# tonyzyl/ladcast

Hardware: AMD Instinct MI355X
Metric: ensemble-member-steps/sec (higher is better)
Workload: dtype f32

## Files before the change

include/ladcast_hip.h:

```cpp
#ifndef LADCAST_HIP_H
#define LADCAST_HIP_H

#ifdef __cplusplus
extern "C" {
#endif

#define LDC_ABI_VERSION 5

#define LDC_OK 0
#define LDC_ERR_ARG (-1)
#define LDC_ERR_ALIGN (-2)
#define LDC_ERR_UNSUPPORTED (-3)

enum ldc_act { LDC_ACT_NONE = 0, LDC_ACT_SILU = 1, LDC_ACT_GELU_TANH = 2, LDC_ACT_RELU = 3 };
#define LDC_ACT_IN_TIMESTEP_SINCOS 16

int ldc_abi_version(void);
const char* ldc_build_arch(void);

typedef struct ldc_gemm_desc {
  int M, N, K, batch;
  int lda, ldw, ldc, ldr;
  long long a_bs, c_bs, r_bs;
  int gate_bs;
// ... 100 lines not shown
int ldc_layernorm_mod(const float* x, float* y, int B, int rows, int D, int ldx, long long x_bs,
                      int ldy, long long y_bs, const float* scale, const float* shift, int mod_bs,
                      int mode, float eps, int out_split, void* stream);
int ldc_layernorm_mod2(const float* x, float* y, int B, int rows, int D, int ldx, long long x_bs,
                       int ldy, long long y_bs, const float* scale, const float* shift, int split_row,
                       const float* scale2, const float* shift2, int mod_bs, int mode, float eps,
                       int out_split, void* stream);

int ldc_mean_rows(const float* x, float* y, int B, int rows, int D, int ldx, long long x_bs, void* stream);
int ldc_mean_rows_split(const float* x, float* y, float* x_split, int B, int rows, int D, int ldx,
                        long long x_bs, int lds, long long s_bs, int fmt , void* stream);

int ldc_gate_residual(const float* resid, const float* y, const float* gate, float* out, int B,
                      int rows, int D, int ld_res, long long res_bs, int ld_y, long long y_bs,
                      int gate_bs, void* stream);
int ldc_gate_residual_layernorm(float* resid, const float* y, const float* gate, float* out, int B, int rows, int D, int ld_res,
                                long long res_bs, int ld_y, long long y_bs, int gate_bs, int ld_out, long long out_bs,
                                const float* weight, const float* bias, float eps, int out_split, void* stream);

int ldc_chan_to_token(const float* in, float* out, int B, int C, int N, int ldo, int fill_cols, void* stream);
int ldc_chan_to_token_split(const float* in, float* out, int B, int C, int N, int ldo, int fill_cols,
                            int out_split, void* stream);
int ldc_token_to_chan(const float* in, float* out, int B, int C, int N, int ldi, void* stream);

int ldc_timestep_embedding(const float* t, float* out, int n, void* stream);

int ldc_temb_modulate(float* temb, const float* te, int B, int D, int te_rows, void* stream);

int ldc_chan_affine(const float* x, float* y, const float* mean, const float* std_, float target_std,
                    long long outer, int C, long long inner, int inverse, void* stream);

int ldc_edm_scale_f64_to_f32(const double* x, double c_in, float* out, long long n, void* stream);
int ldc_edm_init_state(const float* noise, double sigma0, double* x, long long n, void* stream);
int ldc_edm_churn(const double* x_cur, const double* noise, double coef, double* x_hat, long long n, void* stream);
int ldc_edm_euler(const double* x_hat, const float* F, double c_skip, double c_out, double t_hat,
                  double dt, double* x_next, double* d_cur, long long n, void* stream);
int ldc_edm_heun(const double* x_hat, double* x_next, const float* F, const double* d_cur,
                 double c_skip, double c_out, double t_next, double dt, long long n, void* stream);
int ldc_f64_to_f32(const double* x, float* y, long long n, void* stream);
int ldc_dpm_step(const float* sample, const float* F, const float* m1, float* x0, float* prev,
                 float c_skip, float c_out, float a, float b, float inv_r0, int order, long long n,
                 void* stream);
int ldc_ddim_step(const float* sample, const float* F, const float* noise, float* x0, float* prev, float sqrt_alpha_t,
                  float sqrt_beta_t, float sqrt_alpha_prev, float dir_coef, float std_dev, float clip_range,
                  int prediction_type, int use_clipped_model_output, long long n, void* stream);
int ldc_ddpm_step(const float* sample, const float* F, const float* noise, float* x0, float* prev, float sqrt_alpha_t,
// ... 144 lines not shown
```

ladcast_amd/hip.py:

```python
from __future__ import annotations

import ctypes
import os
from ctypes import POINTER, Structure, c_char_p, c_double, c_float, c_int, c_longlong, c_void_p

import torch

_HERE = os.path.dirname(os.path.abspath(__file__))
LIB_PATH = os.environ.get("LDC_LIB_PATH") or os.path.join(_HERE, "libladcast_hip.so")

ACT_NONE, ACT_SILU, ACT_GELU_TANH, ACT_RELU = 0, 1, 2, 3
ACT_IN_TIMESTEP_SINCOS = 16
GEMM_A_SPLIT, GEMM_C_SPLIT, GEMM_BF16_1TERM = 1, 2, 4
GEMM_F32_REGSTAGE = 8
ATTN_OUT_SPLIT, ATTN_BF16_1TERM, ATTN_OUT_BF16 = 1, 2, 4
ABI_VERSION = 5
FMT_F32, FMT_SPLIT, FMT_BF16 = 0, 1, 2


class GemmDesc(Structure):
    _fields_ = [
        ("M", c_int), ("N", c_int), ("K", c_int), ("batch", c_int),
        ("lda", c_int), ("ldw", c_int), ("ldc", c_int), ("ldr", c_int),
        ("a_bs", c_longlong), ("c_bs", c_longlong), ("r_bs", c_longlong),
# ... 86 lines not shown
        "ldc_ensemble_scores_workspace_bytes": (L, [I, I, I]),
        "ldc_ensemble_scores": (I, [P, L, L, P, L, P, L, P, I, I, I, I, I, P, P, P, P, L, P]),
        "ldc_rollout_scores_workspace_bytes": (L, [I, I, I, I]),
        "ldc_rollout_scores": (I, [P, L, L, L, P, P, F, P, L, L, P, P, L, L, P, P, I, I, I, I, I, I, P, I, I, P, L, P]),
        "ldc_validation_scores_workspace_bytes": (L, [I, I, I, I]),
        "ldc_validation_scores": (I, [P, L, L, L, P, P, F, P, L, L, P, P, I, I, I, I, I, P, I, I, P, L, P]),
        "ldc_rollout_reliability_workspace_bytes": (L, [I, I, I, I, I]),
        "ldc_rollout_reliability": (I, [P, L, L, L, P, P, F, P, L, L, P, P, I, I, I, I, I, I, P, P, P, P, I, I, P, L, P]),
        "ldc_rollout_spectrum_workspace_bytes": (L, [I, I, I, I, I]),
        "ldc_rollout_spectrum": (I, [P, L, L, L, P, P, F, P, L, L, P, P, I, I, I, I, I, P, P, I, I, P, L, P]),
        "ldc_sizeof_products_desc": (I, []),
        "ldc_rollout_products": (I, [P, L, L, L, P, P, F, P, I, I, I, I, I, I, POINTER(ProductsDesc), P, P, P, P, I, I, P]),
        "ldc_sizeof_events_desc": (I, []),
        "ldc_rollout_events_workspace_bytes": (L, [I, I, I, I, I]),
        "ldc_rollout_events": (I, [P, L, L, L, P, P, F, P, L, L, P, P, L, L, P, P, I, I, I, I, I, POINTER(EventsDesc), P, P, P, I, I, P, L, P]),
        "ldc_layernorm_mod": (I, [P, P, I, I, I, I, L, I, L, P, P, I, I, F, I, P]),
        "ldc_layernorm_mod2": (I, [P, P, I, I, I, I, L, I, L, P, P, I, P, P, I, I, F, I, P]),
        "ldc_mean_rows": (I, [P, P, I, I, I, I, L, P]),
        "ldc_mean_rows_split": (I, [P, P, P, I, I, I, I, L, I, L, I, P]),
        "ldc_chan_to_token_split": (I, [P, P, I, I, I, I, I, I, P]),
        "ldc_gate_residual": (I, [P, P, P, P, I, I, I, I, L, I, L, I, P]),
        "ldc_chan_to_token": (I, [P, P, I, I, I, I, I, P]),
        "ldc_token_to_chan": (I, [P, P, I, I, I, I, P]),
        "ldc_timestep_embedding": (I, [P, P, I, P]),
        "ldc_temb_modulate": (I, [P, P, I, I, I, P]),
        "ldc_chan_affine": (I, [P, P, P, P, F, L, I, L, I, P]),
        "ldc_edm_scale_f64_to_f32": (I, [P, D, P, L, P]),
        "ldc_edm_init_state": (I, [P, D, P, L, P]),
        "ldc_edm_euler": (I, [P, P, D, D, D, D, P, P, L, P]),
        "ldc_edm_churn": (I, [P, P, c_double, P, L, P]),
        "ldc_edm_heun": (I, [P, P, P, P, D, D, D, D, L, P]),
        "ldc_f64_to_f32": (I, [P, P, L, P]),
        "ldc_dpm_step": (I, [P, P, P, P, P, F, F, F, F, F, I, L, P]),
        "ldc_ddim_step": (I, [P, P, P, P, P, F, F, F, F, F, F, I, I, L, P]),
        "ldc_ddpm_step": (I, [P, P, P, P, P, F, F, F, F, F, F, I, L, P]),
        "ldc_scale_f32": (I, [P, F, P, L, P]),
        "ldc_axpby_f32": (I, [P, F, P, F, P, L, P]),
        "ldc_edm_noise_inputs": (I, [P, P, P, P, P, P, I, L, P]),
        "ldc_edm_denoise": (I, [P, P, P, P, P, I, I, I, I, I, I, I, P]),
        "ldc_edm_denoise_loss": (I, [P, P, P, P, P, P, P, P, P, I, I, I, I, I, P]),
        "ldc_sphere_conv_nhwc": (I, [P, P, P, P, P, I, I, I, I, I, I, I, I, I, I, P]),
        "ldc_sphere_dwconv_nhwc": (I, [P, P, P, P, I, I, I, I, I, I, I, I, P]),
        "ldc_grouped_conv1x1_nhwc": (I, [P, P, P, L, I, I, I, P]),
        "ldc_relu_linear_attn_nhwc": (I, [P, P, I, I, I, I, I, F, P, L, P]),
        "ldc_relu_linear_attn_workspace_bytes": (L, [I, I, I]),
        "ldc_rmsnorm_rows": (I, [P, P, P, P, P, L, I, I, I, I, F, I, P]),
# ... 463 lines not shown
        _check(lib.ldc_mean_rows(_p(x), _p(y), B, rows, D, ldx, x_bs, _stream()), "ldc_mean_rows")
    else:
        _check(lib.ldc_mean_rows_split(_p(x), _p(y), _p(x_split), B, rows, D, ldx, x_bs, lds if lds is not None else ldx,
                                       s_bs if s_bs is not None else x_bs, int(fmt), _stream()), "ldc_mean_rows_split")


def gate_residual(resid, y, gate, out, *, B, rows, D, ld_res, res_bs, ld_y, y_bs, gate_bs):
    _dev(resid, y, gate, out)
    _check(lib.ldc_gate_residual(_p(resid), _p(y), _p(gate), _p(out), B, rows, D, ld_res, res_bs, ld_y, y_bs, gate_bs, _stream()),
           "ldc_gate_residual")


def chan_to_token(x, out, *, B, C, N, ldo, fill_cols=None, out_split=False):
    _dev(x, out)
    _check(lib.ldc_chan_to_token_split(_p(x), _p(out), B, C, N, ldo, ldo if fill_cols is None else fill_cols, int(out_split), _stream()),
           "ldc_chan_to_token")


def token_to_chan(x, out, *, B, C, N, ldi):
    _dev(x, out)
    _check(lib.ldc_token_to_chan(_p(x), _p(out), B, C, N, ldi, _stream()), "ldc_token_to_chan")


def timestep_embedding(t, out, n):
    _dev(t, out)
    _check(lib.ldc_timestep_embedding(_p(t), _p(out), n, _stream()), "ldc_timestep_embedding")


def temb_modulate(temb, te, *, B, D, te_rows):
    _dev(temb, te)
    _check(lib.ldc_temb_modulate(_p(temb), _p(te), B, D, te_rows, _stream()), "ldc_temb_modulate")


def chan_affine(x, y, mean, std, target_std, *, outer, C, inner, inverse):
    _dev(x, y, mean, std)
    _check(lib.ldc_chan_affine(_p(x), _p(y), _p(mean), _p(std), target_std, outer, C, inner, int(inverse), _stream()), "ldc_chan_affine")


TRACK_MAX_CHANNELS, TRACK_MAX_BOXES, TRACK_MAX_INNER, TRACK_MAX_GRID = 8, 8, 30, 1024


def _int_array(values):
    return (c_int * len(values))(*[int(v) for v in values])


def track_gather(x, out, channels, mean, std, *, sb, st, sc, B, T, HW, T_total, t_off, target_std=1.0):
# ... 239 lines not shown
```

ladcast_amd/models/LaDCast_3D_model.py:

```python
from __future__ import annotations

from types import SimpleNamespace
from typing import Optional, Tuple

import numpy as np
import torch
import torch.nn as nn

from .. import graphs, hip
from .embeddings import get_year_sincos_embedding, rope_tables_from_grid, rotary_1d
from .modeling_utils import ModelMixin


class _RMSNormP(nn.Module):
    def __init__(self, dim, eps):
        super().__init__()
        self.eps = eps
        self.weight = nn.Parameter(torch.ones(dim))

    def forward(self, x):
        var = x.to(torch.float32).pow(2).mean(-1, keepdim=True)
        return x * torch.rsqrt(var + self.eps) * self.weight


# ... 524 lines not shown
        C_out = cfg.out_channels or cfg.in_channels
        hidden_states = hidden_states.to(device=dev, dtype=torch.float32).contiguous()
        conditioning_tensors = conditioning_tensors.to(device=dev, dtype=torch.float32)
        if conditioning_tensors.shape[0] != B:
            conditioning_tensors = conditioning_tensors.expand(B, -1, -1, -1, -1)
        conditioning_tensors = conditioning_tensors.contiguous()
        timestep = timestep.to(device=dev, dtype=torch.float32).reshape(-1).contiguous()
        Bt = timestep.shape[0]
        if Bt not in (1, B):
            raise ValueError(f"timestep must have 1 or {B} entries, got {Bt}")
        te = None
        if time_elapsed is not None and self.time_elapsed_embed is not None:
            te = self._time_elapsed_embedding(time_elapsed, dev)
            if te.shape[0] not in (1, B):
                raise ValueError("time_elapsed must have 1 or batch entries")

        if conditioning is not None:
            pack, idx = conditioning
            if tuple(pack.shape) != (B,) + tuple(conditioning_tensors.shape[1:]) or not 0 <= idx < pack.levels:
                raise ValueError("`conditioning` was prepared for another batch / conditioning shape")
            out = self._main_device(hidden_states, pack, idx)
            return (out,) if not return_dict else SimpleNamespace(sample=out)
        if self.use_hip_graph:
            gkey = (B, Bt, C_in, R, T_in, Hh, Ww, None if te is None else (te.data_ptr(), te.shape[0]), bool(self.skip_unread_rows))
            inputs = [hidden_states, timestep, conditioning_tensors]
            ent = self._graphs.get(gkey)
            if ent is None:
                ent = self._graphs[gkey] = graphs.capture(lambda x, t, k: self._forward_device(x, t, k, te), inputs, dev, self.capture_stream())
            out = ent.replay(*inputs)
        else:
            out = self._forward_device(hidden_states, timestep, conditioning_tensors, te)
        if not return_dict:
            return (out,)
        return SimpleNamespace(sample=out)

    def time_elapsed_embedding(self, time_elapsed):
        if time_elapsed is None or self.time_elapsed_embed is None:
            return None
        if self._plan is None:
            self._build_plan()
        return self._time_elapsed_embedding(time_elapsed, self.device)

    def plan_identity(self):
        if self._plan is None:
            self._build_plan()
        return self._plan_gen

    def capture_stream(self):
        if self._capture_stream is None:
            self._capture_stream = torch.cuda.Stream(device=self.device)
        return self._capture_stream

    @torch.no_grad()
    def forward_launch_only(self, hidden_states, timestep, conditioning_tensors, te, conditioning=None):
        if self._plan is None:
            self._build_plan()
        if hidden_states.dtype != torch.float32 or not hidden_states.is_cuda or not hidden_states.is_contiguous():
            raise TypeError("forward_launch_only takes a contiguous fp32 device tensor (use forward() for anything else)")
        if conditioning is not None:
            return self._main_device(hidden_states, conditioning[0], conditioning[1])
        return self._forward_device(hidden_states, timestep.reshape(-1), conditioning_tensors, te)

    batch_conditioning = True
    skip_unread_rows = True
    COND_MAX_ROWS = 96

    @torch.no_grad()
    def prepare_conditioning(self, timesteps, conditioning_tensors, te=None):
        if self._plan is None:
            self._build_plan()
        dev = self.device
        timesteps = timesteps.to(device=dev, dtype=torch.float32).reshape(-1)
        conditioning_tensors = conditioning_tensors.to(device=dev, dtype=torch.float32)
        if conditioning_tensors.dim() != 5:
            raise ValueError("conditioning_tensors must be (B, C, T_in, h, w)")
        N, B = timesteps.shape[0], conditioning_tensors.shape[0]
        shape = tuple(conditioning_tensors.shape)
        per = max(1, self.COND_MAX_ROWS // B)
        if per >= N:
            pk = self._conditioning_device(timesteps.repeat_interleave(B).contiguous(),
                                           conditioning_tensors.unsqueeze(0).expand(N, *shape).reshape(N * B, *shape[1:]).contiguous(), te)
            return SimpleNamespace(ctx=pk.ctx, mods=pk.mods, shape=shape, levels=N)
        Nc, D, NM = shape[2] * shape[3] * shape[4] // self._patch_vol, self.inner_dim, self._plan.mod_w.shape[0]
        key = ("pack", N, B, Nc)
        if key not in self._ws:
            self._ws[key] = (torch.empty(N * B, Nc, D, device=dev, dtype=torch.float32), torch.empty(N * B, NM, device=dev, dtype=torch.float32))
        ctx, mods = self._ws[key]
# ... 126 lines not shown
        cfg = self.config
        D, H = self.inner_dim, cfg.num_attention_heads
        hidden_states = self._patches(hidden_states)
        B, C_in, R, Hh, Ww = hidden_states.shape
        T_in = pack.shape[2] // cfg.patch_size_t
        Nx, Nc = R * Hh * Ww, T_in * Hh * Ww
        S = Nx + Nc
        C_out = (cfg.out_channels or cfg.in_channels) * self._patch_vol
        kpad = max(plan.kx_pad, plan.kc_pad)
        key = (B, Nx, Nc, kpad)
        if key not in self._ws:
            self._ws[key] = _Workspace(dev, B, 1, Nx, Nc, D, kpad, C_out, 4)
        ws = self._ws[key]
        pc, ps, cc, cs, pk, ck, jk = self._rope_tables(R, T_in, Hh, Ww, dev)
        SD = S * D
        h_x, h_c = ws.h[:, :Nx], ws.h[:, Nx:]
        nh_x, nh_c = ws.nh[:, :Nx], ws.nh[:, Nx:]
        NM = plan.mod_w.shape[0]
        mods = pack.mods[idx * B : (idx + 1) * B]
        split = plan.split

        AS, CS, fmt, G, run, run1, run_qkv = self._launchers(plan)

        if split:
            KX = plan.kx_pad
            xtok = ws.xtok.view(-1)[: B * Nx * KX].view(B, Nx, KX)
            hip.chan_to_token(hidden_states, xtok, B=B, C=C_in, N=Nx, ldo=KX, fill_cols=KX, out_split=fmt)
            run1(xtok, plan.wx, h_x, M=Nx, N=D, K=KX, batch=B, a_bs=Nx * KX, c_bs=SD, bias=self.x_embedder.proj.bias, flags=AS)
        else:
            hip.chan_to_token(hidden_states, ws.xtok.view(-1)[: B * Nx * C_in].view(B, Nx, C_in), B=B, C=C_in, N=Nx, ldo=C_in)
            hip.gemm(ws.xtok, plan.wx, h_x, M=Nx, N=D, K=C_in, batch=B, a_bs=Nx * C_in, c_bs=SD, bias=self.x_embedder.proj.bias)
        h_c.copy_(pack.ctx[idx * B : (idx + 1) * B])

        kb_all = None
        if self.scale_attn_by_lat:
            if Hh * Ww != self.attn_lat_weights.numel():
                raise ValueError("scale_attn_by_lat is hard-wired to the 15 x 30 latent grid (models/LaDCast_3D_model.py:684-692)")
            kb_all = self._key_bias(R + T_in, dev)
        foreign = bool(self._foreign_processors())
        m_all = None
        if foreign:
            if split:
                raise NotImplementedError("a user-supplied attention processor runs on the fp32 path: call set_gemm_precision('fp32') "
                                          "(or change the attention arithmetic through the C ABI, include/ladcast_hip.h)")
            if torch.cuda.is_current_stream_capturing():
                raise NotImplementedError("a user-supplied attention processor cannot be captured into a hipGraph")
            if self.scale_attn_by_lat:
                w = self.attn_lat_weights.to(dev)
                m_all = w.repeat(1, 1, 1, T_in + R)


        def mod_of(linear, width):
            o = plan.mod_off[id(linear)]
            return mods[:, o : o + width]

        for blk in self.transformer_blocks:
            pa = plan.attn[id(blk.attn)]
            mx, mc = mod_of(blk.norm1.linear, 6 * D), mod_of(blk.norm1_context.linear, 6 * D)
            hip.layernorm_mod(ws.h, ws.nh, B=B, rows=S, D=D, ldx=D, x_bs=SD, ldy=D, y_bs=SD, scale=mx[:, D:], shift=mx, split_row=Nx, scale2=mc[:, D:], shift2=mc,
                              mod_bs=NM, mode=0, eps=1e-6, out_split=fmt)
            if blk.attn.foreign_processor is not None:
                a, ca = self._call_processor(blk.attn, nh_x, nh_c, m_all, (pc, ps), (cc, cs))
                a, ca = a.contiguous(), ca.contiguous()
                hip.gate_residual(h_x, a, mx[:, 2 * D :], h_x, B=B, rows=Nx, D=D, ld_res=D, res_bs=SD, ld_y=D, y_bs=Nx * D, gate_bs=NM)
                hip.gate_residual(h_c, ca, mc[:, 2 * D :], h_c, B=B, rows=Nc, D=D, ld_res=D, res_bs=SD, ld_y=D, y_bs=Nc * D, gate_bs=NM)
            else:
                nd = run_qkv([
                    G(nh_x, pa.wqkv, ws.qkv, M=Nx, N=3 * D, K=D, batch=B, a_bs=SD, c_bs=S * 3 * D, bias=pa.bqkv, flags=AS),
                    G(nh_c, pa.wqkv_c, ws.qkv[:, Nx:], M=Nc, N=3 * D, K=D, batch=B, a_bs=SD, c_bs=S * 3 * D, bias=pa.bqkv_c, flags=AS),
                ], [self._qkv_epi(blk.attn.norm_q, blk.attn.norm_k, pk), self._qkv_epi(blk.attn.norm_added_q, blk.attn.norm_added_k, None)])
                self._attention(ws, B, 0, Nx, Nc, ws.att, D, SD, (blk.attn.norm_q, blk.attn.norm_k, pc, ps),
                                (blk.attn.norm_added_q, blk.attn.norm_added_k, None, None), out_split=fmt, key_bias=kb_all, normed=nd)
                o, oc = blk.attn.to_out[0], blk.attn.to_add_out
                run([
                    G(ws.att, o.weight, h_x, M=Nx, N=D, K=D, batch=B, a_bs=SD, c_bs=SD, bias=o.bias, gate=mx[:, 2 * D :], gate_bs=NM, R=h_x, ldr=D, r_bs=SD, flags=AS),
                    G(ws.att[:, Nx:], oc.weight, h_c, M=Nc, N=D, K=D, batch=B, a_bs=SD, c_bs=SD, bias=oc.bias, gate=mc[:, 2 * D :], gate_bs=NM, R=h_c, ldr=D, r_bs=SD, flags=AS),
                ])
            hip.layernorm_mod(ws.h, ws.nh, B=B, rows=S, D=D, ldx=D, x_bs=SD, ldy=D, y_bs=SD, scale=mx[:, 4 * D :], shift=mx[:, 3 * D :], split_row=Nx,
                              scale2=mc[:, 4 * D :], shift2=mc[:, 3 * D :], mod_bs=NM, mode=0, eps=1e-7, out_split=fmt)
            up, down = [], []
            for (hs, nhs, rows, ff, mod, off) in ((h_x, nh_x, Nx, blk.ff, mx, 0), (h_c, nh_c, Nc, blk.ff_context, mc, Nx)):
                f0, f2 = ff.net[0].proj, ff.net[2]
                F = f0.weight.shape[0]
# ... 11 lines not shown
            mod = mod_of(blk.norm.linear, 3 * D)
            F = blk.proj_mlp.weight.shape[0]
            W5 = D + F
            cat_mlp = ws.cat.view(torch.bfloat16)[:, :, D:] if plan.one_term else ws.cat[:, :, D:]
            hip.layernorm_mod(ws.h, ws.nh, B=B, rows=S, D=D, ldx=D, x_bs=SD, ldy=D, y_bs=SD, scale=mod[:, D:], shift=mod, mod_bs=NM, mode=0, eps=1e-6, out_split=fmt)
            if blk.attn.foreign_processor is not None:
                run([G(ws.nh, blk.proj_mlp.weight, cat_mlp, M=S, N=F, K=D, batch=B, a_bs=SD, ldc=W5, c_bs=S * W5, bias=blk.proj_mlp.bias,
                       act=hip.ACT_GELU_TANH, flags=AS | CS)])
                a, ca = self._call_processor(blk.attn, ws.nh[:, :Nx], ws.nh[:, Nx:], m_all, (pc, ps), (cc, cs))
                ws.cat[:, :Nx, :D].copy_(a)
                ws.cat[:, Nx:, :D].copy_(ca)
            else:
                nd = run_qkv([
                    G(ws.nh, blk.proj_mlp.weight, cat_mlp, M=Mq, N=F, K=D, batch=B, a_bs=SD, ldc=W5, c_bs=S * W5, bias=blk.proj_mlp.bias, act=hip.ACT_GELU_TANH,
                      flags=AS | CS),
                    G(ws.nh, pa.wqkv, ws.qkv, M=S, N=3 * D, K=D, batch=B, a_bs=SD, c_bs=S * 3 * D, bias=pa.bqkv, flags=AS),
                ], [None, self._qkv_epi(blk.attn.norm_q, blk.attn.norm_k, jk)])
                self._attention(ws, B, 0, Nx, Nc, ws.cat, W5, S * W5, (blk.attn.norm_q, blk.attn.norm_k, pc, ps),
                                (blk.attn.norm_q, blk.attn.norm_k, cc, cs), out_split=fmt, key_bias=kb_all, normed=nd, Sq=None if Mq == S else Mq)
            run1(ws.cat, blk.proj_out.weight, ws.h, M=Mq, N=D, K=W5, batch=B, a_bs=S * W5, c_bs=SD, bias=blk.proj_out.bias,
                        gate=mod[:, 2 * D :], gate_bs=NM, R=ws.h, ldr=D, r_bs=SD, flags=AS)

        mo = mod_of(self.norm_out.linear, 2 * D)
        hip.layernorm_mod(h_x, nh_x, B=B, rows=Nx, D=D, ldx=D, x_bs=SD, ldy=D, y_bs=SD, scale=mo, shift=mo[:, D:], mod_bs=NM, mode=0, eps=1e-7, out_split=fmt)
        run1(nh_x, self.proj_out.weight, ws.otok, M=Nx, N=C_out, K=D, batch=B, a_bs=SD, c_bs=Nx * C_out, bias=self.proj_out.bias, flags=AS)
        out = torch.empty(B, C_out, R, Hh, Ww, device=dev, dtype=torch.float32)
        hip.token_to_chan(ws.otok, out, B=B, C=C_out, N=Nx, ldi=C_out)
        return self._unpatch(out, cfg.out_channels or cfg.in_channels)
```

ladcast_amd/pipelines/edm_sampler.py:

```python
from __future__ import annotations

from typing import List, Optional, Union

import numpy as np
import torch

from .. import graphs, hip
from .torch_utils import randn_tensor


@torch.no_grad()
def edm_AR_sampler(
    net,
    noise_scheduler,
    batch_size=1,
    return_seq_len=1,
    randn_like=torch.randn_like,
    num_inference_steps=18,
    S_churn=0,
    S_min=0,
    S_max=float("inf"),
    S_noise=0,
    deterministic=True,
    known_latents=None,
# ... 13 lines not shown
    shape = (batch_size, net.config.out_channels, return_seq_len, *known_latents.shape[-2:])
    latents = randn_tensor(shape, generator=generator, device=device, dtype=torch.float32).contiguous()
    noise_scheduler.set_timesteps(num_inference_steps, device=device)
    t_steps = noise_scheduler.sigmas
    c_noise_host = noise_scheduler.precondition_noise(t_steps[:-1])
    known = known_latents.to(device=device, dtype=torch.float32)
    if known.shape[0] != batch_size:
        known = known.expand(batch_size, *known.shape[1:])
    known = known.contiguous()

    chunk_graph = bool(getattr(net, "use_hip_graph", False)) and hasattr(net, "forward_launch_only") and hasattr(net, "_graphs")
    batched = bool(getattr(net, "batch_conditioning", False)) and hasattr(net, "prepare_conditioning")
    if not deterministic:
        out = torch.empty(shape, device=device, dtype=torch.float32)
        fwd = lambda x, t, k, te_: net(x, t, k, time_elapsed=timestamps).sample
        _heun_chunk_stochastic(fwd, noise_scheduler, t_steps, latents, known, out, shape, device, num_inference_steps, randn_like, S_churn, S_min,
                               S_max, S_noise)
        return out
    if chunk_graph:
        te = net.time_elapsed_embedding(timestamps)
        plan_id = net.plan_identity()
        key = (tuple(shape), tuple(known.shape), num_inference_steps, tuple(float(v) for v in t_steps.tolist()),
               None if te is None else (te.data_ptr(), tuple(te.shape)), str(device), plan_id, batched,
               bool(getattr(net, "skip_unread_rows", False)))
        prepare = net.prepare_conditioning if batched else None
        key = ("edm_chunk",) + key
        cache = net._graphs
        turn = cache.get(key + ("turn",), 0)
        cache[key + ("turn",)] = turn ^ 1

        def capture():
            st_out, cn = torch.empty(shape, device=device, dtype=torch.float32), c_noise_host.to(device)

            def chunk(lat, kn):
                _heun_chunk(net.forward_launch_only, noise_scheduler, t_steps, cn, lat, kn, te, st_out, shape, device, num_inference_steps, prepare)
                return st_out

            return graphs.capture(chunk, [latents, known], device, net.capture_stream(), keep=cn)

        for inst in (turn, turn ^ 1):
            if cache.get(key + (inst,)) is None:
                cache[key + (inst,)] = capture()
        return cache[key + (turn,)].replay(latents, known)

    out = torch.empty(shape, device=device, dtype=torch.float32)
    c_noise = hip.upload_nonblocking(c_noise_host, device)
    fwd = lambda x, t, k, te_, ci=None: net(x, t, k, time_elapsed=timestamps, **({} if ci is None else {"conditioning": ci})).sample
# ... 60 lines not shown
```

ladcast_amd/pipelines/pipeline_AR.py:

```python
from __future__ import annotations

from typing import List, Optional, Tuple, Union

import torch

from .. import graphs
from .torch_utils import randn_tensor
from .utils import Fields2DPipelineOutput


class AutoRegressive2DPipeline:
    model_cpu_offload_seq = "unet"

    def __init__(self, ar_model, scheduler, scheduler_step_kwargs: Optional[dict] = None):
        self.register_modules(ar_model=ar_model, scheduler=scheduler)
        self.scheduler_step_kwargs = scheduler_step_kwargs or {}

    def register_modules(self, **mods):
        for k, v in mods.items():
            setattr(self, k, v)

    @property
    def _execution_device(self):
        return self.ar_model.device
# ... 45 lines not shown
        pack = None
        if getattr(net, "batch_conditioning", False) and hasattr(net, "prepare_conditioning"):
            kn = known_latents if known_latents.shape[0] == batch_size else known_latents.expand(batch_size, *known_latents.shape[1:])
            pack = net.prepare_conditioning(self.scheduler.timesteps, kn.contiguous(), net.time_elapsed_embedding(timestamps))
        for i, t in enumerate(self.scheduler.timesteps):
            if not do_edm_style:
                raise NotImplementedError("Only EDM style is supported for now")
            x_in = self.scheduler.scale_model_input(image, t)
            t_host = t
            t = t.expand(batch_size).to(dev)
            t.host_value = t_host
            ckw = {} if pack is None else {"conditioning": (pack, i)}
            model_output = self.ar_model(x_in, t, known_latents, time_elapsed=timestamps, return_dict=False, **ckw)[0]
            image = self.scheduler.step(model_output, t, image, **self.scheduler_step_kwargs, return_dict=False)[0]
        if not return_dict:
            return (image,)
        return Fields2DPipelineOutput(fields=image)

    def _graph_loop(self, net, sch, image, known, timestamps, num_inference_steps, batch_size, dev):
        sch.set_timesteps(num_inference_steps)
        te = net.time_elapsed_embedding(timestamps)
        key = (tuple(image.shape), tuple(known.shape), num_inference_steps, sch.graph_signature(),
               tuple(sorted((k, str(v)) for k, v in self.scheduler_step_kwargs.items())), None if te is None else (te.data_ptr(), tuple(te.shape)), str(dev), net.plan_identity(),
               bool(getattr(net, "batch_conditioning", False)), bool(getattr(net, "skip_unread_rows", False)))
        key = ("pipeline_loop",) + key
        cache = net._graphs
        ent = cache.get(key)
        if ent is None:
            ts_dev = sch.timesteps.to(device=dev, dtype=torch.float32).contiguous()
            tsteps = [t.to(device=dev, dtype=torch.float32).expand(batch_size).contiguous() for t in sch.timesteps]

            def loop(img, kn):
                kb = kn if kn.shape[0] == batch_size else kn.expand(batch_size, *kn.shape[1:]).contiguous()
                pack = net.prepare_conditioning(ts_dev, kb, te) if getattr(net, "batch_conditioning", False) else None
                for i, (t, t_dev) in enumerate(zip(sch.timesteps, tsteps)):
                    x_in = sch.scale_model_input(img, t)
                    out = net.forward_launch_only(x_in, t_dev, kb, te, None if pack is None else (pack, i))
                    img = sch.step(out, t, img, **self.scheduler_step_kwargs, return_dict=False)[0]
                return img

            ent = graphs.capture(loop, [image, known], dev, net.capture_stream(), reset=lambda: sch.set_timesteps(num_inference_steps),
                                 keep={"tsteps": tsteps, "ts_dev": ts_dev})
            ent.keep["scheduler_state"] = sch.graph_state()
            cache[key] = ent
        out = ent.replay(image, known)
        sch.set_graph_state(ent.keep["scheduler_state"])
        return out
# ... 1 lines not shown
```

Baseline: 3.219.

## Fuse token embedding with first layernorm and head layernorm with output projection

Adds two HIP kernels. The first does the input channel-to-token transpose, the embedding GEMM with bias, the context copy and the first block's modulated layernorm in one launch. The second fuses the final modulated layernorm, the output projection and the token-to-channel transpose. The aim is to cut several kernel launches and intermediate global-memory round trips at the model's edges. The price is custom MFMA code with shape limits, falling back to the old path when unsupported, and the graph cache keys now include the new flag.

```diff
diff --git a/include/ladcast_hip.h b/include/ladcast_hip.h
--- a/include/ladcast_hip.h
+++ b/include/ladcast_hip.h
@@ -146,6 +146,13 @@
 int ldc_chan_to_token_split(const float* in, float* out, int B, int C, int N, int ldo, int fill_cols,
                             int out_split, void* stream);
 int ldc_token_to_chan(const float* in, float* out, int B, int C, int N, int ldi, void* stream);
+
+int ldc_embed_tokens_ln(const float* x, const float* W, const float* bias, const float* ctx, float* h, float* nh, int B,
+                        int C_in, int Nx, int Nc, int D, int ldh, long long h_bs, int ldn, long long n_bs, int ldc,
+                        long long c_bs, const float* scale, const float* shift, const float* scale2, const float* shift2,
+                        int mod_bs, int mode, float eps, void* stream);
+int ldc_head_ln_proj(const float* hx, const float* W, const float* bias, float* out, int B, int Nx, int D, int C_out, int ldx,
+                     long long x_bs, const float* scale, const float* shift, int mod_bs, float eps, void* stream);
 
 int ldc_timestep_embedding(const float* t, float* out, int n, void* stream);
 
diff --git a/ladcast_amd/csrc/forward_edges.hip b/ladcast_amd/csrc/forward_edges.hip
--- /dev/null
+++ b/ladcast_amd/csrc/forward_edges.hip
@@ -0,0 +1,362 @@
+#include "common.h"
+
+namespace {
+
+constexpr int FE_ROWS = 16;
+constexpr int FE_WAVES = 8;
+constexpr int FE_THREADS = 64 * FE_WAVES;
+constexpr int FE_MAX_V4 = 8;
+constexpr int FE_KMAX = 128;
+constexpr int FE_PRE = 16 * FE_KMAX / 64;
+constexpr int FE_CT_MAX = 6;
+constexpr int FE_HG = 3;
+
+struct FeMod {
+  const float* scale;
+  const float* shift;
+  const float* scale2;
+  const float* shift2;
+  int mod_bs;
+  int mode;
+  float eps;
+};
+
+__device__ __forceinline__ void fe_load_row(const float* __restrict__ xr, int nv4, int lane, float4 (&v)[FE_MAX_V4]) {
+#pragma unroll
+  for (int i = 0; i < FE_MAX_V4; ++i) {
+    const int c = lane + 64 * i;
+    v[i] = c < nv4 ? reinterpret_cast<const float4*>(xr)[c] : make_float4(0.f, 0.f, 0.f, 0.f);
+  }
+}
+__device__ __forceinline__ void fe_row_stats(const float4 (&v)[FE_MAX_V4], int nv4, int lane, int D, float eps, float& mean, float& rstd) {
+  float sum = 0.f;
+#pragma unroll
+  for (int i = 0; i < FE_MAX_V4; ++i)
+    if (lane + 64 * i < nv4) sum += (v[i].x + v[i].y) + (v[i].z + v[i].w);
+  mean = wave_sum(sum) / static_cast<float>(D);
+  float sq = 0.f;
+#pragma unroll
+  for (int i = 0; i < FE_MAX_V4; ++i)
+    if (lane + 64 * i < nv4) {
+      const float a = v[i].x - mean, bq = v[i].y - mean, cq = v[i].z - mean, dq = v[i].w - mean;
+      sq += (a * a + bq * bq) + (cq * cq + dq * dq);
+    }
+  rstd = rsqrtf(wave_sum(sq) / static_cast<float>(D) + eps);
+}
+__device__ __forceinline__ float4 fe_modulate(float4 v, float mean, float rstd, const float* __restrict__ sc, const float* __restrict__ sh,
+                                              int c, float one) {
+  const float4 m = sc ? reinterpret_cast<const float4*>(sc)[c] : make_float4(1.f - one, 1.f - one, 1.f - one, 1.f - one);
+  const float4 a = sh ? reinterpret_cast<const float4*>(sh)[c] : make_float4(0.f, 0.f, 0.f, 0.f);
+  float4 o;
+  o.x = (v.x - mean) * rstd * (one + m.x) + a.x;
+  o.y = (v.y - mean) * rstd * (one + m.y) + a.y;
+  o.z = (v.z - mean) * rstd * (one + m.z) + a.z;
+  o.w = (v.w - mean) * rstd * (one + m.w) + a.w;
+  return o;
+}
+
+__device__ __forceinline__ void fe_fetch_tile(const float* __restrict__ W, long long first, long long count, int n_here, int lane,
+                                              float (&pre)[FE_PRE]) {
+#pragma unroll
+  for (int j = 0; j < FE_PRE; ++j) {
+    const int idx = 64 * j + lane;
+    pre[j] = (idx < n_here && first + idx < count) ? W[first + idx] : 0.f;
+  }
+}
+
+template <int N>
+__device__ __forceinline__ void fe_embed_steps(const float* __restrict__ wa, const float* __restrict__ xb, int s, int klim, f32x4& acc) {
+  float a[N], bv[N];
+#pragma unroll
+  for (int i = 0; i < N; ++i) {
+    a[i] = (4 * (s + i) < klim) ? wa[4 * (s + i)] : 0.f;
+    bv[i] = xb[4 * (s + i) * FE_ROWS];
+  }
+#pragma unroll
+  for (int i = 0; i < N; ++i) acc = __builtin_amdgcn_mfma_f32_16x16x4f32(a[i], bv[i], acc, 0, 0, 0);
+}
+
+__global__ __launch_bounds__(FE_THREADS) void embed_tokens_ln_kernel(const float* __restrict__ x, const float* __restrict__ W,
+                                                                     const float* __restrict__ bias, const float* __restrict__ ctx,
+                                                                     float* __restrict__ h, float* __restrict__ nh, int C, int Nx, int Nc,
+                                                                     int D, int ldh, long long h_bs, int ldn, long long n_bs, int ldc,
+                                                                     long long c_bs, FeMod m) {
+  extern __shared__ __attribute__((aligned(16))) float smem[];
+  const int lane = threadIdx.x & 63, wave = threadIdx.x >> 6;
+  const int b = blockIdx.y;
+  const int nxb = (Nx + FE_ROWS - 1) / FE_ROWS;
+  const int nv4 = D >> 2;
+  const float one = (m.mode == 0) ? 1.f : 0.f;
+  const long long mod_off = m.mode == 0 ? static_cast<long long>(b) * m.mod_bs : 0;
+
+  if (static_cast<int>(blockIdx.x) >= nxb) {
+    const float* sc = m.scale2 ? m.scale2 + mod_off : nullptr;
+    const float* sh = m.shift2 ? m.shift2 + mod_off : nullptr;
+#pragma unroll 1
+    for (int q = 0; q < FE_ROWS / FE_WAVES; ++q) {
+      const int rc = (static_cast<int>(blockIdx.x) - nxb) * FE_ROWS + wave * (FE_ROWS / FE_WAVES) + q;
+      if (rc >= Nc) break;
+      float* hr = h + b * h_bs + static_cast<long long>(Nx + rc) * ldh;
+      float* yr = nh + b * n_bs + static_cast<long long>(Nx + rc) * ldn;
+      float4 v[FE_MAX_V4];
+      fe_load_row(ctx ? ctx + b * c_bs + static_cast<long long>(rc) * ldc : hr, nv4, lane, v);
+      if (ctx) {
+#pragma unroll
+        for (int i = 0; i < FE_MAX_V4; ++i)
+          if (lane + 64 * i < nv4) reinterpret_cast<float4*>(hr)[lane + 64 * i] = v[i];
+      }
+      float mean, rstd;
+      fe_row_stats(v, nv4, lane, D, m.eps, mean, rstd);
+#pragma unroll
+      for (int i = 0; i < FE_MAX_V4; ++i) {
+        const int c = lane + 64 * i;
+        if (c < nv4) reinterpret_cast<float4*>(yr)[c] = fe_modulate(v[i], mean, rstd, sc, sh, c, one);
+      }
+    }
+    return;
+  }
+
+  const int r0 = blockIdx.x * FE_ROWS;
+  const int col = lane & 15, kq = lane >> 4;
+  const int KP = (C + 3) & ~3, nks = KP >> 2;
+  const int tile_f = FE_ROWS * C, ldr = D + 4;
+  float* xs = smem;
+  float* wt = smem + KP * FE_ROWS + wave * tile_f;
+  float* rows = smem + KP * FE_ROWS + FE_WAVES * tile_f;
+  for (int idx = threadIdx.x; idx < KP * FE_ROWS; idx += FE_THREADS) {
+    const int k = idx >> 4, j = idx & 15;
+    xs[idx] = (k < C && r0 + j < Nx) ? x[(static_cast<long long>(b) * C + k) * Nx + r0 + j] : 0.f;
+  }
+  const int ntiles = (D + 15) >> 4;
+  const int tpw = (ntiles + FE_WAVES - 1) / FE_WAVES;
+  const long long w_count = static_cast<long long>(D) * C;
+  auto tile_floats = [&](int tg) {
+    const int rows_w = D - 16 * tg;
+    return tg < ntiles ? (rows_w < 16 ? rows_w : 16) * C : 0;
+  };
+  float pre[FE_PRE];
+  fe_fetch_tile(W, static_cast<long long>(wave * tpw) * tile_f, w_count, tile_floats(wave * tpw), lane, pre);
+  const float* wa = wt + col * C + kq;
+  const float* xb = xs + kq * FE_ROWS + col;
+#pragma unroll 1
+  for (int t = 0; t < tpw; ++t) {
+    const int tg = wave * tpw + t;
+#pragma unroll
+    for (int j = 0; j < FE_PRE; ++j)
+      if (64 * j + lane < tile_f) wt[64 * j + lane] = pre[j];
+    __syncthreads();
+    if (t + 1 < tpw) fe_fetch_tile(W, static_cast<long long>(tg + 1) * tile_f, w_count, tile_floats(tg + 1), lane, pre);
+    const int d = 16 * tg + 4 * kq;
+    if (d < D) {
+      f32x4 acc = f32x4{0.f, 0.f, 0.f, 0.f};
+      int s = 0;
+      for (; s + 8 <= nks; s += 8) fe_embed_steps<8>(wa, xb, s, C - kq, acc);
+      if (s + 4 <= nks) { fe_embed_steps<4>(wa, xb, s, C - kq, acc); s += 4; }
+      for (; s < nks; ++s) fe_embed_steps<1>(wa, xb, s, C - kq, acc);
+      float4 v = make_float4(acc[0], acc[1], acc[2], acc[3]);
+      if (bias) {
+        const float4 bv = *reinterpret_cast<const float4*>(bias + d);
+        v.x += bv.x; v.y += bv.y; v.z += bv.z; v.w += bv.w;
+      }
+      *reinterpret_cast<float4*>(rows + col * ldr + d) = v;
+    }
+    __syncthreads();
+  }
+  const float* sc = m.scale ? m.scale + mod_off : nullptr;
+  const float* sh = m.shift ? m.shift + mod_off : nullptr;
+#pragma unroll
+  for (int q = 0; q < FE_ROWS / FE_WAVES; ++q) {
+    const int j = wave * (FE_ROWS / FE_WAVES) + q, r = r0 + j;
+    if (r >= Nx) continue;
+    float4 v[FE_MAX_V4];
+    fe_load_row(rows + j * ldr, nv4, lane, v);
+    float* hr = h + b * h_bs + static_cast<long long>(r) * ldh;
+    float* yr = nh + b * n_bs + static_cast<long long>(r) * ldn;
+    float mean, rstd;
+    fe_row_stats(v, nv4, lane, D, m.eps, mean, rstd);
+#pragma unroll
+    for (int i = 0; i < FE_MAX_V4; ++i) {
+      const int c = lane + 64 * i;
+      if (c < nv4) {
+        reinterpret_cast<float4*>(hr)[c] = v[i];
+        reinterpret_cast<float4*>(yr)[c] = fe_modulate(v[i], mean, rstd, sc, sh, c, one);
+      }
+    }
+  }
+}
+
+__global__ __launch_bounds__(FE_THREADS) void head_ln_proj_kernel(const float* __restrict__ hx, int ldx, long long x_bs,
+                                                                  const float* __restrict__ W, const float* __restrict__ bias,
+                                                                  float* __restrict__ out, int Nx, int D, int Co,
+                                                                  const float* __restrict__ scale, const float* __restrict__ shift,
+                                                                  int mod_bs, float eps) {
+  extern __shared__ __attribute__((aligned(16))) float smem[];
+  const int lane = threadIdx.x & 63, wave = threadIdx.x >> 6;
+  const int col = lane & 15, kq = lane >> 4;
+  const int b = blockIdx.y;
+  const int r0 = blockIdx.x * FE_ROWS;
+  const int nv4 = D >> 2, ldn = D + 4;
+  const float* sc = scale ? scale + static_cast<long long>(b) * mod_bs : nullptr;
+  const float* sh = shift ? shift + static_cast<long long>(b) * mod_bs : nullptr;
+  {
+    constexpr int RPW = FE_ROWS / FE_WAVES;
+    float4 v[RPW][FE_MAX_V4];
+#pragma unroll
+    for (int q = 0; q < RPW; ++q) {
+      const int j = wave * RPW + q;
+      if (r0 + j < Nx) fe_load_row(hx + b * x_bs + static_cast<long long>(r0 + j) * ldx, nv4, lane, v[q]);
+    }
+#pragma unroll
+    for (int q = 0; q < RPW; ++q) {
+      const int j = wave * RPW + q;
+      float* nr = smem + j * ldn;
+      if (r0 + j < Nx) {
+        float mean, rstd;
+        fe_row_stats(v[q], nv4, lane, D, eps, mean, rstd);
+#pragma unroll
+        for (int i = 0; i < FE_MAX_V4; ++i) {
+          const int c = lane + 64 * i;
+          if (c < nv4) reinterpret_cast<float4*>(nr)[c] = fe_modulate(v[q][i], mean, rstd, sc, sh, c, 1.f);
+        }
+      } else {
+        for (int c = lane; c < nv4; c += 64) reinterpret_cast<float4*>(nr)[c] = make_float4(0.f, 0.f, 0.f, 0.f);
+      }
+    }
+  }
+  __syncthreads();
+
+  const int ctiles = (Co + 15) >> 4;
+  const int nu = D >> 4;
+  const int per = (nu + FE_WAVES - 1) / FE_WAVES;
+  const int u0 = wave * per, u1 = u0 + per < nu ? u0 + per : nu;
+  f32x4 acc[FE_CT_MAX];
+#pragma unroll
+  for (int ct = 0; ct < FE_CT_MAX; ++ct) acc[ct] = f32x4{0.f, 0.f, 0.f, 0.f};
+  const float* wrow[FE_CT_MAX];
+  bool wok[FE_CT_MAX];
+#pragma unroll
+  for (int ct = 0; ct < FE_CT_MAX; ++ct) {
+    const int c = 16 * ct + col;
+    wok[ct] = ct < ctiles && c < Co;
+    wrow[ct] = W + static_cast<long long>(wok[ct] ? c : 0) * D + 4 * kq;
+  }
+  const float* nb = smem + col * ldn + 4 * kq;
+  f32x4 wc[FE_HG][FE_CT_MAX], wn[FE_HG][FE_CT_MAX];
+  auto fetch = [&](int u, f32x4 (&dst)[FE_HG][FE_CT_MAX]) {
+#pragma unroll
+    for (int g = 0; g < FE_HG; ++g)
+#pragma unroll
+      for (int ct = 0; ct < FE_CT_MAX; ++ct)
+        if (ct < ctiles && u + g < u1) {
+          const f32x4 t = *reinterpret_cast<const f32x4*>(wrow[ct] + 16 * (u + g));
+          dst[g][ct] = wok[ct] ? t : f32x4{0.f, 0.f, 0.f, 0.f};
+        }
+  };
+  if (u0 < u1) fetch(u0, wc);
+  for (int u = u0; u < u1; u += FE_HG) {
+    if (u + FE_HG < u1) fetch(u + FE_HG, wn);
+#pragma unroll
+    for (int g = 0; g < FE_HG; ++g)
+      if (u + g < u1) {
+        const float4 bv = *reinterpret_cast<const float4*>(nb + 16 * (u + g));
+#pragma unroll
+        for (int ct = 0; ct < FE_CT_MAX; ++ct)
+          if (ct < ctiles) {
+            acc[ct] = __builtin_amdgcn_mfma_f32_16x16x4f32(wc[g][ct][0], bv.x, acc[ct], 0, 0, 0);
+            acc[ct] = __builtin_amdgcn_mfma_f32_16x16x4f32(wc[g][ct][1], bv.y, acc[ct], 0, 0, 0);
+            acc[ct] = __builtin_amdgcn_mfma_f32_16x16x4f32(wc[g][ct][2], bv.z, acc[ct], 0, 0, 0);
+            acc[ct] = __builtin_amdgcn_mfma_f32_16x16x4f32(wc[g][ct][3], bv.w, acc[ct], 0, 0, 0);
+          }
+      }
+    if (u + FE_HG < u1) {
+#pragma unroll
+      for (int g = 0; g < FE_HG; ++g)
+#pragma unroll
+        for (int ct = 0; ct < FE_CT_MAX; ++ct) wc[g][ct] = wn[g][ct];
+    }
+  }
+  __syncthreads();
+  const int cw = 16 * ctiles;
+#pragma unroll
+  for (int ct = 0; ct < FE_CT_MAX; ++ct)
+    if (ct < ctiles) {
+#pragma unroll
+      for (int i = 0; i < 4; ++i) smem[(wave * cw + 16 * ct + 4 * kq + i) * FE_ROWS + col] = acc[ct][i];
+    }
+  __syncthreads();
+  float* ob = out + static_cast<long long>(b) * Co * Nx;
+  for (int idx = threadIdx.x; idx < cw * FE_ROWS; idx += FE_THREADS) {
+    const int c = idx >> 4, j = idx & 15;
+    if (c >= Co || r0 + j >= Nx) continue;
+    float s = 0.f;
+#pragma unroll
+    for (int w = 0; w < FE_WAVES; ++w) s += smem[(w * cw + c) * FE_ROWS + j];
+    ob[static_cast<long long>(c) * Nx + r0 + j] = s + (bias ? bias[c] : 0.f);
+  }
+}
+
+constexpr int FE_LDS_MAX = 160 * 1024;
+
+}
+
+extern "C" int ldc_embed_tokens_ln(const float* x, const float* W, const float* bias, const float* ctx, float* h, float* nh, int B,
+                                   int C_in, int Nx, int Nc, int D, int ldh, long long h_bs, int ldn, long long n_bs, int ldc,
+                                   long long c_bs, const float* scale, const float* shift, const float* scale2, const float* shift2,
+                                   int mod_bs, int mode, float eps, void* stream) {
+  LDC_CHECK_PTR(x);
+  LDC_CHECK_PTR(W);
+  LDC_CHECK_PTR(h);
+  LDC_CHECK_PTR(nh);
+  if (B <= 0 || C_in <= 0 || Nx <= 0 || Nc < 0 || D <= 0) return LDC_ERR_ARG;
+  if (ldh < D || ldn < D || (ctx && ldc < D)) return LDC_ERR_ARG;
+  if (h == nh) return LDC_ERR_ARG;
+  if ((D & 3) || D > 64 * 4 * FE_MAX_V4 || C_in > FE_KMAX || B > 65535) return LDC_ERR_UNSUPPORTED;
+  if (mode != 0 && mode != 1) return LDC_ERR_UNSUPPORTED;
+  if ((ldh & 3) || (ldn & 3) || (h_bs & 3) || (n_bs & 3) || (mod_bs & 3) || (ctx && ((ldc & 3) || (c_bs & 3)))) return LDC_ERR_ALIGN;
+  LDC_CHECK_ALIGN16(h);
+  LDC_CHECK_ALIGN16(nh);
+  if (bias) LDC_CHECK_ALIGN16(bias);
+  if (ctx) LDC_CHECK_ALIGN16(ctx);
+  if (scale) LDC_CHECK_ALIGN16(scale);
+  if (shift) LDC_CHECK_ALIGN16(shift);
+  if (scale2) LDC_CHECK_ALIGN16(scale2);
+  if (shift2) LDC_CHECK_ALIGN16(shift2);
+  const int KP = (C_in + 3) & ~3;
+  const int lds = (KP * FE_ROWS + FE_WAVES * FE_ROWS * C_in + FE_ROWS * (D + 4)) * static_cast<int>(sizeof(float));
+  if (lds > FE_LDS_MAX) return LDC_ERR_UNSUPPORTED;
+  static const bool attr_set = [] {
+    (void)hipFuncSetAttribute(reinterpret_cast<const void*>(embed_tokens_ln_kernel), hipFuncAttributeMaxDynamicSharedMemorySize, FE_LDS_MAX);
+    return true;
+  }();
+  (void)attr_set;
+  const FeMod m{scale, shift, scale2, shift2, mod_bs, mode, eps};
+  dim3 grid(ldc_cdiv(Nx, FE_ROWS) + ldc_cdiv(Nc, FE_ROWS), B);
+  hipLaunchKernelGGL(embed_tokens_ln_kernel, grid, dim3(FE_THREADS), lds, static_cast<hipStream_t>(stream), x, W, bias, ctx, h, nh, C_in, Nx, Nc, D,
+                     ldh, h_bs, ldn, n_bs, ldc, c_bs, m);
+  return ldc_launch_status();
+}
+
+extern "C" int ldc_head_ln_proj(const float* hx, const float* W, const float* bias, float* out, int B, int Nx, int D, int C_out, int ldx,
+                                long long x_bs, const float* scale, const float* shift, int mod_bs, float eps, void* stream) {
+  LDC_CHECK_PTR(hx);
+  LDC_CHECK_PTR(W);
+  LDC_CHECK_PTR(out);
+  if (B <= 0 || Nx <= 0 || D <= 0 || C_out <= 0 || ldx < D) return LDC_ERR_ARG;
+  if ((D & 15) || D > 64 * 4 * FE_MAX_V4 || C_out > 16 * FE_CT_MAX || B > 65535) return LDC_ERR_UNSUPPORTED;
+  if ((ldx & 3) || (x_bs & 3) || (mod_bs & 3)) return LDC_ERR_ALIGN;
+  LDC_CHECK_ALIGN16(hx);
+  LDC_CHECK_ALIGN16(W);
+  if (scale) LDC_CHECK_ALIGN16(scale);
+  if (shift) LDC_CHECK_ALIGN16(shift);
+  const int ctiles = ldc_cdiv(C_out, 16);
+  const int f_rows = FE_ROWS * (D + 4), f_part = FE_WAVES * 16 * ctiles * FE_ROWS;
+  const int lds = (f_rows > f_part ? f_rows : f_part) * static_cast<int>(sizeof(float));
+  static const bool attr_set = [] {
+    (void)hipFuncSetAttribute(reinterpret_cast<const void*>(head_ln_proj_kernel), hipFuncAttributeMaxDynamicSharedMemorySize, FE_LDS_MAX);
+    return true;
+  }();
+  (void)attr_set;
+  hipLaunchKernelGGL(head_ln_proj_kernel, dim3(ldc_cdiv(Nx, FE_ROWS), B), dim3(FE_THREADS), lds, static_cast<hipStream_t>(stream), hx, ldx, x_bs,
+                     W, bias, out, Nx, D, C_out, scale, shift, mod_bs, eps);
+  return ldc_launch_status();
+}
diff --git a/ladcast_amd/hip.py b/ladcast_amd/hip.py
--- a/ladcast_amd/hip.py
+++ b/ladcast_amd/hip.py
@@ -132,6 +132,8 @@
         "ldc_gate_residual": (I, [P, P, P, P, I, I, I, I, L, I, L, I, P]),
         "ldc_chan_to_token": (I, [P, P, I, I, I, I, I, P]),
         "ldc_token_to_chan": (I, [P, P, I, I, I, I, P]),
+        "ldc_embed_tokens_ln": (I, [P, P, P, P, P, P, I, I, I, I, I, I, L, I, L, I, L, P, P, P, P, I, I, F, P]),
+        "ldc_head_ln_proj": (I, [P, P, P, P, I, I, I, I, I, L, P, P, I, F, P]),
         "ldc_timestep_embedding": (I, [P, P, I, P]),
         "ldc_temb_modulate": (I, [P, P, I, I, I, P]),
         "ldc_chan_affine": (I, [P, P, P, P, F, L, I, L, I, P]),
@@ -641,6 +643,26 @@
     _check(lib.ldc_token_to_chan(_p(x), _p(out), B, C, N, ldi, _stream()), "ldc_token_to_chan")
 
 
+def embed_tokens_ln(x, W, bias, ctx, h, nh, *, B, C_in, Nx, Nc, D, ldh, h_bs, ldn, n_bs, ldc=0, c_bs=0, scale=None, shift=None, scale2=None,
+                    shift2=None, mod_bs=0, mode=0, eps=1e-6):
+    _dev(x, W, bias, ctx, h, nh, scale, shift, scale2, shift2)
+    rc = lib.ldc_embed_tokens_ln(_p(x), _p(W), _p(bias), _p(ctx), _p(h), _p(nh), B, C_in, Nx, Nc, D, ldh, h_bs, ldn, n_bs, ldc, c_bs, _p(scale),
+                                 _p(shift), _p(scale2), _p(shift2), mod_bs, mode, eps, _stream())
+    if rc == ERR_UNSUPPORTED:
+        return False
+    _check(rc, "ldc_embed_tokens_ln")
+    return True
+
+
+def head_ln_proj(hx, W, bias, out, *, B, Nx, D, C_out, ldx, x_bs, scale=None, shift=None, mod_bs=0, eps=1e-6):
+    _dev(hx, W, bias, out, scale, shift)
+    rc = lib.ldc_head_ln_proj(_p(hx), _p(W), _p(bias), _p(out), B, Nx, D, C_out, ldx, x_bs, _p(scale), _p(shift), mod_bs, eps, _stream())
+    if rc == ERR_UNSUPPORTED:
+        return False
+    _check(rc, "ldc_head_ln_proj")
+    return True
+
+
 def timestep_embedding(t, out, n):
     _dev(t, out)
     _check(lib.ldc_timestep_embedding(_p(t), _p(out), n, _stream()), "ldc_timestep_embedding")
diff --git a/ladcast_amd/models/LaDCast_3D_model.py b/ladcast_amd/models/LaDCast_3D_model.py
--- a/ladcast_amd/models/LaDCast_3D_model.py
+++ b/ladcast_amd/models/LaDCast_3D_model.py
@@ -570,7 +570,7 @@
             out = self._main_device(hidden_states, pack, idx)
             return (out,) if not return_dict else SimpleNamespace(sample=out)
         if self.use_hip_graph:
-            gkey = (B, Bt, C_in, R, T_in, Hh, Ww, None if te is None else (te.data_ptr(), te.shape[0]), bool(self.skip_unread_rows))
+            gkey = (B, Bt, C_in, R, T_in, Hh, Ww, None if te is None else (te.data_ptr(), te.shape[0]), bool(self.skip_unread_rows), bool(self.fused_edges))
             inputs = [hidden_states, timestep, conditioning_tensors]
             ent = self._graphs.get(gkey)
             if ent is None:
@@ -611,6 +611,7 @@
 
     batch_conditioning = True
     skip_unread_rows = True
+    fused_edges = True
     COND_MAX_ROWS = 96
 
     @torch.no_grad()
@@ -783,7 +784,17 @@
 
         AS, CS, fmt, G, run, run1, run_qkv = self._launchers(plan)
 
-        if split:
+        fused = bool(self.fused_edges) and not split and self._patch_vol == 1 and not self._foreign_processors()
+        normed0 = False
+        if fused and len(self.transformer_blocks):
+            b0 = self.transformer_blocks[0]
+            o_x, o_c = plan.mod_off[id(b0.norm1.linear)], plan.mod_off[id(b0.norm1_context.linear)]
+            normed0 = hip.embed_tokens_ln(hidden_states, plan.wx, self.x_embedder.proj.bias, pack.ctx[idx * B : (idx + 1) * B], ws.h, ws.nh, B=B, C_in=C_in,
+                                          Nx=Nx, Nc=Nc, D=D, ldh=D, h_bs=SD, ldn=D, n_bs=SD, ldc=D, c_bs=Nc * D, scale=mods[:, o_x + D :], shift=mods[:, o_x:],
+                                          scale2=mods[:, o_c + D :], shift2=mods[:, o_c:], mod_bs=NM, mode=0, eps=1e-6)
+        if normed0:
+            pass
+        elif split:
             KX = plan.kx_pad
             xtok = ws.xtok.view(-1)[: B * Nx * KX].view(B, Nx, KX)
             hip.chan_to_token(hidden_states, xtok, B=B, C=C_in, N=Nx, ldo=KX, fill_cols=KX, out_split=fmt)
@@ -791,7 +802,8 @@
         else:
             hip.chan_to_token(hidden_states, ws.xtok.view(-1)[: B * Nx * C_in].view(B, Nx, C_in), B=B, C=C_in, N=Nx, ldo=C_in)
             hip.gemm(ws.xtok, plan.wx, h_x, M=Nx, N=D, K=C_in, batch=B, a_bs=Nx * C_in, c_bs=SD, bias=self.x_embedder.proj.bias)
-        h_c.copy_(pack.ctx[idx * B : (idx + 1) * B])
+        if not normed0:
+            h_c.copy_(pack.ctx[idx * B : (idx + 1) * B])
 
         kb_all = None
         if self.scale_attn_by_lat:
@@ -815,11 +827,12 @@
             o = plan.mod_off[id(linear)]
             return mods[:, o : o + width]
 
-        for blk in self.transformer_blocks:
+        for i_blk, blk in enumerate(self.transformer_blocks):
             pa = plan.attn[id(blk.attn)]
             mx, mc = mod_of(blk.norm1.linear, 6 * D), mod_of(blk.norm1_context.linear, 6 * D)
-            hip.layernorm_mod(ws.h, ws.nh, B=B, rows=S, D=D, ldx=D, x_bs=SD, ldy=D, y_bs=SD, scale=mx[:, D:], shift=mx, split_row=Nx, scale2=mc[:, D:], shift2=mc,
-                              mod_bs=NM, mode=0, eps=1e-6, out_split=fmt)
+            if not (normed0 and i_blk == 0):
+                hip.layernorm_mod(ws.h, ws.nh, B=B, rows=S, D=D, ldx=D, x_bs=SD, ldy=D, y_bs=SD, scale=mx[:, D:], shift=mx, split_row=Nx, scale2=mc[:, D:],
+                                  shift2=mc, mod_bs=NM, mode=0, eps=1e-6, out_split=fmt)
             if blk.attn.foreign_processor is not None:
                 a, ca = self._call_processor(blk.attn, nh_x, nh_c, m_all, (pc, ps), (cc, cs))
                 a, ca = a.contiguous(), ca.contiguous()
@@ -877,8 +890,10 @@
                         gate=mod[:, 2 * D :], gate_bs=NM, R=ws.h, ldr=D, r_bs=SD, flags=AS)
 
         mo = mod_of(self.norm_out.linear, 2 * D)
-        hip.layernorm_mod(h_x, nh_x, B=B, rows=Nx, D=D, ldx=D, x_bs=SD, ldy=D, y_bs=SD, scale=mo, shift=mo[:, D:], mod_bs=NM, mode=0, eps=1e-7, out_split=fmt)
-        run1(nh_x, self.proj_out.weight, ws.otok, M=Nx, N=C_out, K=D, batch=B, a_bs=SD, c_bs=Nx * C_out, bias=self.proj_out.bias, flags=AS)
         out = torch.empty(B, C_out, R, Hh, Ww, device=dev, dtype=torch.float32)
-        hip.token_to_chan(ws.otok, out, B=B, C=C_out, N=Nx, ldi=C_out)
+        if not (fused and hip.head_ln_proj(h_x, self.proj_out.weight, self.proj_out.bias, out, B=B, Nx=Nx, D=D, C_out=C_out, ldx=D, x_bs=SD, scale=mo,
+                                           shift=mo[:, D:], mod_bs=NM, eps=1e-7)):
+            hip.layernorm_mod(h_x, nh_x, B=B, rows=Nx, D=D, ldx=D, x_bs=SD, ldy=D, y_bs=SD, scale=mo, shift=mo[:, D:], mod_bs=NM, mode=0, eps=1e-7, out_split=fmt)
+            run1(nh_x, self.proj_out.weight, ws.otok, M=Nx, N=C_out, K=D, batch=B, a_bs=SD, c_bs=Nx * C_out, bias=self.proj_out.bias, flags=AS)
+            hip.token_to_chan(ws.otok, out, B=B, C=C_out, N=Nx, ldi=C_out)
         return self._unpatch(out, cfg.out_channels or cfg.in_channels)
diff --git a/ladcast_amd/pipelines/edm_sampler.py b/ladcast_amd/pipelines/edm_sampler.py
--- a/ladcast_amd/pipelines/edm_sampler.py
+++ b/ladcast_amd/pipelines/edm_sampler.py
@@ -59,7 +59,8 @@
         plan_id = net.plan_identity()
         key = (tuple(shape), tuple(known.shape), num_inference_steps, tuple(float(v) for v in t_steps.tolist()),
                None if te is None else (te.data_ptr(), tuple(te.shape)), str(device), plan_id, batched,
-               bool(getattr(net, "skip_unread_rows", False)))
+               bool(getattr(net, "skip_unread_rows", False)),
+               bool(getattr(net, "fused_edges", False)))
         prepare = net.prepare_conditioning if batched else None
         key = ("edm_chunk",) + key
         cache = net._graphs
diff --git a/ladcast_amd/pipelines/pipeline_AR.py b/ladcast_amd/pipelines/pipeline_AR.py
--- a/ladcast_amd/pipelines/pipeline_AR.py
+++ b/ladcast_amd/pipelines/pipeline_AR.py
@@ -91,7 +91,8 @@
         te = net.time_elapsed_embedding(timestamps)
         key = (tuple(image.shape), tuple(known.shape), num_inference_steps, sch.graph_signature(),
                tuple(sorted((k, str(v)) for k, v in self.scheduler_step_kwargs.items())), None if te is None else (te.data_ptr(), tuple(te.shape)), str(dev), net.plan_identity(),
-               bool(getattr(net, "batch_conditioning", False)), bool(getattr(net, "skip_unread_rows", False)))
+               bool(getattr(net, "batch_conditioning", False)), bool(getattr(net, "skip_unread_rows", False)),
+               bool(getattr(net, "fused_edges", False)))
         key = ("pipeline_loop",) + key
         cache = net._graphs
         ent = cache.get(key)
```

Measured after the change: 3.216. No clear change (-0.1%).
